# lblQubic/distributed_processor

Hardware: AMD Instinct MI355X
Metric: emulated core-shots/s (config 2: 8-core Ramsey, 100 delays, 1e6 shots/GPU) (higher is better)
Workload: dtype u32; 1 GPU; config2_ramsey_8core_100pt; shots_per_gpu=1000000, lane_order=shot-major, parallelism=shots sharded, 1 GPU(s)

## Files before the change

### distributed_processor_amd/csrc/branch_kernel.h

```cpp

#pragma once

#include <hip/hip_runtime.h>
#include <stdint.h>

#include <type_traits>

#include "lane.h"

namespace dpemu {

namespace {

enum : uint32_t { B_RUN = 0, B_SYNC = 1, B_LUT = 2, B_FIN = 3 };


constexpr uint64_t LATENCY = 0x0003303304646440ull;

template <int OP>
__device__ __forceinline__ uint32_t group_reduce(uint32_t v, uint32_t C)
{
    auto comb = [](uint32_t a, uint32_t b) { return OP == 0 ? (a < b ? a : b) : (a > b ? a : b); };
#define DPP(x, ctrl) ((uint32_t)__builtin_amdgcn_update_dpp(0, (int)(x), (ctrl), 0xF, 0xF, false))
    if (C >= 2) v = comb(v, DPP(v, 0xB1));
    if (C >= 4) v = comb(v, DPP(v, 0x4E));
    if (C >= 8) v = comb(v, DPP(v, 0x141));
    if (C >= 16) v = comb(v, DPP(v, 0x140));
#undef DPP
    for (uint32_t m = 16; m < C; m <<= 1) v = comb(v, (uint32_t)__shfl_xor((int)v, (int)m, 64));
    return v;
}

__device__ __forceinline__ uint32_t wave_min(uint32_t v)
{
    v = group_reduce<0>(v, 16u);
    const uint32_t a = __builtin_amdgcn_readlane(v, 0), b = __builtin_amdgcn_readlane(v, 16);
    const uint32_t c = __builtin_amdgcn_readlane(v, 32), d = __builtin_amdgcn_readlane(v, 48);
    return min(min(a, b), min(c, d));
}

}

template <int FEAT, int CT>
__global__ void __launch_bounds__(BLOCK) branch_kernel(const KParams p)
{
    constexpr bool FPROC = (FEAT & FEAT_FPROC) != 0;
    constexpr bool LUT = (FEAT & FEAT_LUT) != 0;
    constexpr bool XMEAS = FPROC || LUT;
    constexpr bool SYNC = (FEAT & FEAT_SYNC) != 0;
    constexpr bool REGS = (FEAT & FEAT_REGS) != 0;
    constexpr bool PLDS = (FEAT & FEAT_PROG_LDS) != 0;
    constexpr bool DEMOD = (FEAT & FEAT_DEMOD) != 0;
    constexpr int MT = XMEAS ? MEAS_LOOKUP : 1;
    constexpr bool DIRECT = LUT || DEMOD;
    constexpr int NF = LUT ? LUT_FIRE_CAP : 1;

    __shared__ uint32_t s_regs[REGS ? 16 : 1][REGS ? BLOCK : 1];
    __shared__ uint32_t s_mt[MT][BLOCK];
    __shared__ uint32_t s_fire[NF][LUT ? BLOCK : 1];
    __shared__ uint32_t s_pref[PLDS ? BLOCK + 1 : 1];
    __shared__ uint32_t s_scan[BLOCK / 64];
    __shared__ uint32_t s_rof[DEMOD ? 6 : 1][DEMOD ? BLOCK : 1];
    extern __shared__ uint4 s_dyn[];
    uint4 *const s_prog = s_dyn;
    uint32_t *const s_hist = reinterpret_cast<uint32_t *>(s_dyn + (PLDS ? p.prog_lds_words : 0u));

    clear_hist_next(p);
    const uint32_t tid = threadIdx.x;
    const uint32_t C = CT ? (uint32_t)CT : p.C;
    const uint32_t log2C = CT ? (uint32_t)__builtin_ctz(CT) : p.log2C;
    const uint32_t pos = blockIdx.x * BLOCK + tid;
    const bool valid = pos < p.n_lanes;
    const uint32_t core = pos & (C - 1);
    const uint32_t spos = pos >> log2C;
    const uint32_t lane = out_lane(p, spos, core);
    const uint64_t shot = p.shot_begin + spos;
    const uint32_t wl = tid & 63;
    const uint32_t leader_tid = tid & ~(C - 1);
    const uint32_t n_lanes = p.n_lanes, max_cycles = p.max_cycles;

    uint32_t nprog = 0, grp = 0, prog = 0, base = 0;
    if (valid) {
        grp = shot_group(p, spos);
        prog = p.prog_table[(uint64_t)grp * C + core];
        base = p.offsets[prog];
        nprog = p.n_instr[prog];
    }
    if constexpr (PLDS) {
        const uint32_t b = stage_programs(p, s_prog, s_pref, s_scan, spos, core);
        if (valid) base = b;
    }
    const bool cmd_major = !PLDS && p.fetch_stride != 1u;
    const uint32_t fetch_off = cmd_major ? prog : base, k_max = cmd_major ? p.max_len : nprog;
    const uint32_t thr_core = valid ? p.p1_thr[core] : 0u;
    if constexpr (DEMOD) {
        const uint4 h = valid ? p.ro_hdr[prog] : make_uint4(0u, 0u, 0u, 0u);
        s_rof[0][tid] = h.x; s_rof[1][tid] = h.y; s_rof[2][tid] = h.z; s_rof[3][tid] = h.w;
        s_rof[4][tid] = ro_freq(p, h.x, h.y, 0u);
        s_rof[5][tid] = ro_freq(p, h.z, h.w, 0u);
    }
    if (p.hist_lds) {
        for (uint32_t i = tid; i < HIST_LDS_MAX; i += BLOCK) s_hist[i] = 0;
        __syncthreads();
    }
    if constexpr (REGS) {
#pragma unroll
        for (int r = 0; r < 16; r++) s_regs[r][tid] = 0;
    }
    if constexpr (XMEAS) {
#pragma unroll
        for (int m = 0; m < MT; m++) s_mt[m][tid] = INF32;
    }
    uint64_t lut_valid = 0, lut_addr = 0;
    uint32_t lut_last_fire = INF32, nfire = 0, lut_cur = 0;

    uint32_t mode = valid ? B_RUN : B_FIN;
    uint32_t ip = 0, t = 0, qoff = 0xFFFFFFFFu;
    uint32_t pe = 0, pp = 0, pa = 0;
    uint32_t wait_d = 0, status = 0, flags = 0, t_end = 0;
    uint32_t n_ev = 0, n_tr = 0, n_meas = 0, n_exec = 0, meas_bits = 0, last_bit = 0;
    const bool is_part = SYNC ? (((p.sync_mask >> core) & 1ull) != 0) : false;
    uint4 *const ev_lane = p.events + lane;
    uint4 pend0 = make_uint4(0u, 0u, 0u, 0u), pend1 = pend0;
    uint32_t n_st = 0;
    RoDrive ro_d{0u, 0u, 0u};
    uint32_t ro_tref = 0, ro_ltv = 0;

    auto emit = [&](bool ok, uint32_t te, uint32_t kind) __attribute__((always_inline)) {
        if (ok) {
            if (DIRECT && n_ev < p.event_cap && p.events)
                st_rec<ST_WB>(&ev_lane[(uint64_t)n_ev * n_lanes], event_record(te, pe, pp, pa, kind));
            if (!DIRECT && n_ev < p.event_cap && p.events) {
                const uint4 rec = event_record(te, pe, pp, pa, kind);
                const bool full = n_ev - n_st == 2u;
                if (full) st_rec<ST_WB>(&ev_lane[(uint64_t)n_st * n_lanes], pend0);
                pend0 = sel4(full, pend1, pend0);
                n_st += full ? 1u : 0u;
                const bool first = n_ev == n_st;
                pend0 = sel4(first, rec, pend0);
                pend1 = sel4(first, pend1, rec);
            }
            n_ev++;
            if constexpr (DEMOD) {
                if (kind == 1u) ro_tref = te;
                if (kind == 0u && ((pe >> 24) & 3u) == p.ro_drv_elem)
                    ro_d = RoDrive{te, pp & 0x03FFFFFFu, (pa & 0xFFFFu) | (((pe >> 12) & 0xFFFu) << 16) | 0x80000000u};
            }
            if (kind == 0u && ((pe >> 24) & 3u) == p.meas_elem) {
                uint32_t bit, tv;
                if constexpr (DEMOD) {
                    int2 a;
                    const uint32_t fi_lo = (pp >> 17) & 0x1FFu, fi_d = (ro_d.pp >> 17) & 0x1FFu;
                    const uint32_t f_lo = fi_lo ? ro_freq(p, s_rof[2][tid], s_rof[3][tid], fi_lo) : s_rof[5][tid];
                    const uint32_t f_d = fi_d ? ro_freq(p, s_rof[0][tid], s_rof[1][tid], fi_d) : s_rof[4][tid];
                    bit = demod_readout(p, shot, core, n_meas, thr_core, te, pe, pp, ro_d, ro_tref, f_lo, f_d, a);
                    tv = demod_valid(p, te, pe, ro_ltv);
                    ro_ltv = tv;
                    if (p.acc && n_meas < p.meas_cap) p.acc[(uint64_t)n_meas * n_lanes + lane] = a;
                } else {
                    bit = meas_bit(p, shot, core, n_meas, thr_core, pa, pe);
                    tv = te + p.meas_latency;
                }
                if constexpr (XMEAS) {
                    if (n_meas < (uint32_t)MT) s_mt[n_meas < (uint32_t)MT ? n_meas : 0u][tid] = (tv << 1) | bit;
                }
                if (p.meas && n_meas < p.meas_cap) p.meas[(uint64_t)n_meas * n_lanes + lane] = make_uint2(tv, bit);
                meas_bits |= (n_meas < 32u ? bit : 0u) << (n_meas & 31u);
                last_bit = bit;
                n_meas++;
            }
        }
    };

    auto emit_trace = [&](bool ok, uint32_t tt, uint32_t addr, uint32_t val) __attribute__((always_inline)) {
        if (ok) {
            if (n_tr < p.trace_cap && p.trace) p.trace[(uint64_t)n_tr * n_lanes + lane] = make_uint4(tt, addr, val, 0u);
            n_tr++;
        }
    };

    auto meas_lookup = [&](uint32_t q_tid, uint32_t d) -> uint32_t {
        static_assert(MEAS_LOOKUP % 2 == 0, "slots read in pairs");
        uint32_t res = 0;
#pragma unroll 1
        for (int m = 0; m + 1 < MT; m += 2) {
            const uint32_t e0 = s_mt[m][q_tid], e1 = s_mt[m + 1][q_tid];
            if ((e0 >> 1) > d) break;
            res = e0 & 1u;
            if ((e1 >> 1) > d) break;
            res = e1 & 1u;
        }
        return res;
    };

    auto sync_maxkey = [&]() -> uint32_t {
        uint32_t key = mode == B_SYNC ? wait_d : t;
        if constexpr (LUT) key = mode == B_LUT ? wait_d + 5u : key;
        key = mode == B_FIN ? INF32 : key;
        return group_reduce<1>(is_part ? key : 0u, C);
    };

    auto reg = [&](uint32_t r) __attribute__((always_inline)) -> uint32_t {
        if constexpr (REGS) return s_regs[r & 15u][tid];
        return 0u;
    };

    auto finish = [&](bool stop, uint32_t st, uint32_t at) __attribute__((always_inline)) {
        status = stop ? st : status;
        t_end = stop ? at : t_end;
        mode = stop ? B_FIN : mode;
    };

    auto flush_rows = [&](bool all) __attribute__((always_inline)) {
        if (DIRECT || !p.events) return;
        const uint32_t ne = min(n_ev, p.event_cap);
        if (!__any(ne > n_st)) return;
        const uint32_t done = all ? INF32 : wave_min(mode == B_FIN ? INF32 : ne);
        const bool f1 = n_st < ne && n_st < done;
        if (!__any(f1)) return;
        const bool f2 = f1 && n_st + 1u < ne && n_st + 1u < done;
        if (f1) st_rec<ST_WB>(&ev_lane[(uint64_t)n_st * n_lanes], pend0);
        if (__any(f2)) {
            if (f2) st_rec<ST_WB>(&ev_lane[(uint64_t)(n_st + 1u) * n_lanes], pend1);
        }
        pend0 = sel4(f1 && !f2, pend1, pend0);
        n_st += (f1 ? 1u : 0u) + (f2 ? 1u : 0u);
    };

    auto iteration = [&](auto first_tag) -> bool {
        constexpr bool FIRST = decltype(first_tag)::value;
        finish(mode == B_RUN && t > max_cycles, ST_MAX_CYCLES, t);
        const bool run = mode == B_RUN;
        const uint4 u = PLDS ? s_prog[fetch_off + min(ip, k_max)]
                             : p.fetch[(uint64_t)min(ip, k_max) * p.fetch_stride + fetch_off];
        const uint32_t op = u.y >> 28;

        bool stall = false;
        if constexpr (FPROC) {
            const bool fp = run && (op == 4u || op == 5u);
            if (__any(fp)) {
                uint32_t bound = run ? t + 2u : INF32;
                if constexpr (SYNC) {
                    if (__any(mode == B_SYNC)) {
                        const uint32_t maxkey = sync_maxkey();
                        if (mode == B_SYNC && is_part && maxkey != INF32) bound = maxkey + p.sync_latency + 5u;
                    }
                }
                const uint32_t gmin = group_reduce<0>(bound, C);
                stall = fp && !((uint64_t)gmin + p.meas_latency > (uint64_t)t);
            }
        }
        const bool go = run && !stall;
        bool sync_rel = false;
        n_exec += go ? 1u : 0u;
        const uint32_t D = t;
        const uint32_t qD = FIRST ? 0u : D + qoff;

        constexpr uint32_t FAST = 0xFF05u | (SYNC ? 0x80u : 0u);
        const bool pcls = (FAST >> op) & 1u;
        {
            const bool pg = go && pcls;
            const bool waits = (0x1200u >> op) & 1u;
            uint32_t wait = u.x - qD;
            bool big = false, dbl = false;
            if constexpr (FIRST) {
                dbl = u.x == 0u;
                const uint64_t w = dbl ? 0ull : 1ull + u.x;
                wait = (uint32_t)w;
                big = (w >> 32) != 0ull;
            }
            const bool late = waits && (big || wait >= 0x80000000u);
            const bool over = waits && (big || wait > max_cycles - D);
            const uint32_t tT = D + (waits ? wait : 0u);
            const bool jmp = op == 2u;
            const bool to_sync = SYNC && pg && op == 7u;
            const bool cont = pg && (((0x1B04u >> op) & 1u) != 0u) && !over;
            if (__any(cont && ((0x300u >> op) & 1u))) {
                uint32_t pe2 = pe, pp2 = pp, pa2 = pa;
                pulse_write(u, pe2, pp2, pa2);
                if (cont && (u.w & UOP_ANY_RS)) {
                    const uint32_t r0 = reg(u.w >> 20);
                    if (u.w & UOP_RS_ENV) pe2 |= r0 & 0xFFFFFFu;
                    if (u.w & UOP_RS_PH) pp2 |= r0 & 0x1FFFFu;
                    if (u.w & UOP_RS_FR) pp2 |= (r0 & 0x1FFu) << 17;
                    if (u.w & UOP_RS_AMP) pa2 = r0 & 0xFFFFu;
                }
                pe = cont ? pe2 : pe;
                pp = cont ? pp2 : pp;
                pa = cont ? pa2 : pa;
            }
            const bool rst = op == 0xBu;
            emit(cont && (op == 9u || rst), rst ? D : tT + 2u, rst ? 1u : 0u);
            if constexpr (FIRST) {
                const bool two = cont && dbl && op == 9u;
                emit(two, tT + 3u, 0u);
                flags |= two ? F_DOUBLE_STROBE : 0u;
            }
            flags |= (pg && late) ? F_LATE : 0u;
            if (__any(pg && !cont && !to_sync)) {
                finish(pg && !cont && !to_sync, over ? ST_MAX_CYCLES : op >= 0xDu ? ST_HUNG_OPCODE : ST_DONE, D);
            }
            wait_d = to_sync ? D : wait_d;
            mode = to_sync ? B_SYNC : mode;
            ip = cont ? (jmp ? (u.z & 0xFFFFu) : ((ip + 1u) & 0xFFFFu)) : ip;
            t = cont ? (jmp ? D + 4u : tT + 3u) : t;
        }
        if (__any(go && !pcls)) {
            const bool sg = go && !pcls;
            const bool is_fp = op == 4u || op == 5u;
            const uint32_t reg0 = reg(u.w >> 20);
            const uint32_t reg1 = reg(u.y >> 4);
            uint32_t data = 0;
            uint32_t R = D + 2u;
            bool lut_wait = false, no_meas = false;
            if constexpr (FPROC) {
                if (__any(sg && is_fp)) {
                    if (sg && is_fp) data = meas_lookup(leader_tid + (((u.z >> 16) & 0xFFu) & (C - 1u)), D);
                }
            }
            if constexpr (LUT) {
                if (__any(sg && is_fp)) {
                    const bool id0 = ((u.z >> 16) & 0xFFu) == 0u;
                    lut_wait = sg && is_fp && !id0;
                    if (sg && is_fp && id0) {
                        uint32_t e = INF32;
#pragma unroll
                        for (int m = MT - 1; m >= 0; m--) {
                            const uint32_t x = s_mt[m][tid];
                            e = (x != INF32 && (x >> 1) >= D + 1u) ? x : e;
                        }
                        no_meas = e == INF32;
                        R = e >> 1;
                        data = e & 1u;
                    }
                }
            }
            const uint32_t in0 = (u.y & 8u) ? reg0 : u.x;
            const uint32_t out = alu_eval(u.y & 7u, in0, op == 6u ? qD : is_fp ? data : reg1);
            const bool absent = (!XMEAS && is_fp) || (!SYNC && op == 7u);
            const bool r_over = XMEAS && is_fp && !lut_wait && !no_meas && R > max_cycles;
            const bool fin = r_over || absent || no_meas;
            const bool cont = sg && !fin;
            const bool to_sync = SYNC && cont && op == 7u;
            const bool to_lut = LUT && cont && lut_wait;
            const bool adv = cont && !to_sync && !to_lut;
            const uint32_t t_next = (is_fp ? R : D) + (uint32_t)((LATENCY >> (4u * op)) & 15u);
            const bool take = op == 2u || ((op == 3u || op == 5u) && (out & 1u));
            const uint32_t ip_next = take ? (u.z & 0xFFFFu) : ((ip + 1u) & 0xFFFFu);
            const bool wr = adv && (op == 1u || op == 4u);
            if constexpr (REGS) {
                if (wr) s_regs[(u.y >> 8) & 15u][tid] = out;
            }
            const bool inc = adv && op == 6u;
            emit_trace(wr || inc, (op == 4u ? R : D) + 3u, inc ? TRACE_QCLK_LOAD : (u.y >> 8) & 15u,
                       inc ? out + 3u : out);
            qoff = inc ? out - D : qoff;
            finish(sg && fin, r_over ? ST_MAX_CYCLES : ST_DEADLOCK, D);
            wait_d = (to_sync || to_lut) ? D : wait_d;
            mode = to_sync ? B_SYNC : to_lut ? B_LUT : mode;
            ip = adv ? ip_next : ip;
            t = adv ? t_next : t;
        }

        if constexpr (SYNC) {
            if (__any(mode == B_SYNC)) {
                const uint32_t maxkey = sync_maxkey();
                const uint64_t b = __ballot(is_part && mode == B_SYNC);
                const uint64_t pm = __ballot(is_part);
                const bool all_arrived = group_bits(b, wl, C) == group_bits(pm, wl, C) && group_bits(pm, wl, C) != 0ull;
                const bool rel = mode == B_SYNC && is_part && all_arrived;
                const uint32_t S = maxkey + p.sync_latency;
                const bool ok = rel && S <= max_cycles;
                emit_trace(ok, S + 2u, TRACE_QCLK_RST, 0u);
                qoff = ok ? 0u - (S + 2u) : qoff;
                ip = ok ? ((ip + 1u) & 0xFFFFu) : ip;
                t = ok ? S + 3u : t;
                mode = ok ? B_RUN : mode;
                finish(rel && !ok, ST_MAX_CYCLES, wait_d);
                sync_rel = rel;
                if constexpr (!LUT)
                    finish(group_bits(__ballot(go || rel), wl, C) == 0ull && mode == B_SYNC, ST_DEADLOCK, wait_d);
            }
        }

        bool lut_rel = false;
        if constexpr (LUT) {
            __builtin_amdgcn_fence(__ATOMIC_SEQ_CST, "wavefront");
            __builtin_amdgcn_wave_barrier();
            if (__any(mode == B_LUT)) {
                uint32_t bound = mode == B_RUN ? t + 2u : mode == B_LUT ? wait_d + 7u : INF32;
                if constexpr (SYNC) {
                    if (__any(mode == B_SYNC)) {
                        const uint32_t maxkey = sync_maxkey();
                        if (mode == B_SYNC && is_part && maxkey != INF32) bound = maxkey + p.sync_latency + 5u;
                    }
                }
                const uint32_t gmin = group_reduce<0>(bound, C);
                const bool any_run_grp = group_bits(__ballot(mode == B_RUN), wl, C) != 0ull;
                uint32_t H = INF32;
                if (any_run_grp && gmin != INF32) {
                    const uint64_t h = (uint64_t)gmin + p.meas_latency - 1u;
                    H = h > INF32 ? INF32 : (uint32_t)h;
                }
                const bool stop_at_fire = !any_run_grp;
                bool fired = false, busy = valid;
                while (__any(busy)) {
                    const uint32_t e = lut_cur < (uint32_t)MT ? s_mt[lut_cur < (uint32_t)MT ? lut_cur : 0u][tid] : INF32;
                    const uint32_t my = e == INF32 ? INF32 : e >> 1;
                    const uint32_t tmin = group_reduce<0>(my, C);
                    busy = busy && tmin != INF32 && tmin <= H;
                    const bool hit = busy && my == tmin;
                    const uint64_t v = group_bits(__ballot(hit), wl, C);
                    const uint64_t mv = group_bits(__ballot(hit && (e & 1u)), wl, C);
                    lut_cur += hit ? 1u : 0u;
                    const bool upd = busy && !(lut_last_fire != INF32 && tmin == lut_last_fire + 1u);
                    const uint64_t nv = lut_valid | v, na = lut_addr | (v & mv);
                    const bool fire = upd && (((uint64_t)p.lut_mask & nv) == (uint64_t)p.lut_mask);
                    if (fire) {
                        if (nfire < (uint32_t)NF) {
                            const uint64_t o = p.lut_table[na & 0xFFu];
                            s_fire[nfire < (uint32_t)NF ? nfire : 0u][tid] = (tmin << 1) | (uint32_t)((o >> core) & 1ull);
                        }
                        lut_last_fire = tmin;
                        nfire++;
                        fired = true;
                    }
                    lut_valid = fire ? 0ull : upd ? nv : lut_valid;
                    lut_addr = fire ? 0ull : upd ? na : lut_addr;
                    busy = busy && !(fire && stop_at_fire);
                }
                const uint32_t nf_grp = nfire;
                const bool grp_fired = fired;
                __builtin_amdgcn_fence(__ATOMIC_SEQ_CST, "wavefront");
                __builtin_amdgcn_wave_barrier();
                if (mode == B_LUT) {
                    const uint32_t n = nf_grp < (uint32_t)NF ? nf_grp : (uint32_t)NF;
                    for (uint32_t k = 0; k < n; k++) {
                        const uint32_t f = s_fire[k][tid], tf = f >> 1;
                        if (tf >= wait_d + 1u) {
                            const uint4 u2 = PLDS ? s_prog[fetch_off + min(ip, k_max)]
                                                  : p.fetch[(uint64_t)min(ip, k_max) * p.fetch_stride + fetch_off];
                            const uint32_t op2 = u2.y >> 28;
                            const uint32_t in0b = (u2.y & 8u) ? reg(u2.w >> 20) : u2.x;
                            const uint32_t outb = alu_eval(u2.y & 7u, in0b, f & 1u);
                            if (tf > max_cycles) {
                                finish(true, ST_MAX_CYCLES, wait_d);
                            } else if (op2 == 4u) {
                                const uint32_t rd = (u2.y >> 8) & 15u;
                                if constexpr (REGS) s_regs[rd][tid] = outb;
                                emit_trace(true, tf + 3u, rd, outb);
                                ip = (ip + 1u) & 0xFFFFu;
                                t = tf + 4u;
                                mode = B_RUN;
                            } else {
                                ip = (outb & 1u) ? (u2.z & 0xFFFFu) : ((ip + 1u) & 0xFFFFu);
                                t = tf + 6u;
                                mode = B_RUN;
                            }
                            lut_rel = true;
                            break;
                        }
                    }
                }
                lut_rel = lut_rel || (grp_fired && tid == leader_tid);
            }
            if (__any(mode == B_SYNC || mode == B_LUT)) {
                const uint64_t pm = __ballot(go || sync_rel || lut_rel);
                finish(group_bits(pm, wl, C) == 0ull && (mode == B_SYNC || mode == B_LUT), ST_DEADLOCK, wait_d);
            }
        }
        if constexpr (XMEAS) {
            __builtin_amdgcn_fence(__ATOMIC_SEQ_CST, "wavefront");
            __builtin_amdgcn_wave_barrier();
        }
        flush_rows(false);
        return __any(mode != B_FIN);
    };

    if (__any(mode != B_FIN) && iteration(std::true_type{})) {
        for (uint32_t iter = 2; iteration(std::false_type{});) {
            if (++iter > p.iter_guard) {
                flags |= mode != B_FIN ? F_GUARD : 0u;
                finish(mode != B_FIN, ST_DEADLOCK, t);
                break;
            }
        }
    }
    flush_rows(true);
    flags |= (n_ev > p.event_cap ? F_EVENT_OVF : 0u) | (n_meas > min(p.meas_cap, MEAS_LOOKUP) ? F_MEAS_OVF : 0u) |
             ((p.trace_cap && n_tr > p.trace_cap) ? F_TRACE_OVF : 0u);

    if (valid && p.summary) {
        const uint32_t qclk_end = t_end == 0u ? 0u : t_end + qoff;
        write_summary(p, lane, t_end, ip, status, flags, n_ev, n_exec, qclk_end, n_meas, meas_bits, n_tr);
    }
    if (valid && p.regs_out) {
#pragma unroll
        for (int r = 0; r < 16; r++) p.regs_out[(uint64_t)r * n_lanes + lane] = reg(r);
    }
    count_outcome(p, s_hist, valid, core, grp, last_bit);
}

template <int F>
static hipError_t launch_branch_f(const KParams &p, uint32_t blocks, hipStream_t stream)
{
    const size_t shmem = ((F & FEAT_PROG_LDS) ? (size_t)p.prog_lds_words * sizeof(uint4) : 0) +
                         (p.hist_lds ? HIST_LDS_MAX * sizeof(uint32_t) : 0);
    if (p.C == 8) hipLaunchKernelGGL((branch_kernel<F, 8>), dim3(blocks), dim3(BLOCK), shmem, stream, p);
    else hipLaunchKernelGGL((branch_kernel<F, 0>), dim3(blocks), dim3(BLOCK), shmem, stream, p);
    return hipGetLastError();
}

}
```

Measured before the change: 55.43 billion core-shots/s.

## Execute up to three fast-class instructions per interpreter iteration

Moves the fast-opcode handling into a reusable lambda and, after the main step, runs up to two extra fast-path instructions for lanes that just continued, so each loop iteration advances more instructions and spends less on per-iteration overhead (finish checks, sync/LUT handling, wave votes). It also narrows the LUT valid/address bitmasks to 32 bits when the core count fits. The cost is larger code and register use plus extra divergence-vote checks, and lanes that finish their extra slots early sit idle while others keep going.

Result: no change. 55.43 billion core-shots/s (median of 4 runs) (+0.0%).

```diff
diff --git a/distributed_processor_amd/csrc/branch_kernel.h b/distributed_processor_amd/csrc/branch_kernel.h
--- a/distributed_processor_amd/csrc/branch_kernel.h
+++ b/distributed_processor_amd/csrc/branch_kernel.h
@@ -54,6 +54,8 @@
     constexpr int MT = XMEAS ? MEAS_LOOKUP : 1;
     constexpr bool DIRECT = LUT || DEMOD;
     constexpr int NF = LUT ? LUT_FIRE_CAP : 1;
+    constexpr uint32_t FAST = 0xFF05u | (SYNC ? 0x80u : 0u);
+    constexpr int SLOTS = 3;
 
     __shared__ uint32_t s_regs[REGS ? 16 : 1][REGS ? BLOCK : 1];
     __shared__ uint32_t s_mt[MT][BLOCK];
@@ -111,7 +113,8 @@
 #pragma unroll
         for (int m = 0; m < MT; m++) s_mt[m][tid] = INF32;
     }
-    uint64_t lut_valid = 0, lut_addr = 0;
+    using lut_bits_t = std::conditional_t<(CT > 0 && CT <= 32), uint32_t, uint64_t>;
+    lut_bits_t lut_valid = 0, lut_addr = 0;
     uint32_t lut_last_fire = INF32, nfire = 0, lut_cur = 0;
 
     uint32_t mode = valid ? B_RUN : B_FIN;
@@ -227,6 +230,56 @@
         n_st += (f1 ? 1u : 0u) + (f2 ? 1u : 0u);
     };
 
+    auto fast_path = [&](auto first_tag, const uint4 u, const uint32_t op, bool pg, uint32_t D,
+                         uint32_t qD) __attribute__((always_inline)) -> bool {
+        constexpr bool FIRST = decltype(first_tag)::value;
+        const bool waits = (0x1200u >> op) & 1u;
+        uint32_t wait = u.x - qD;
+        bool big = false, dbl = false;
+        if constexpr (FIRST) {
+            dbl = u.x == 0u;
+            const uint64_t w = dbl ? 0ull : 1ull + u.x;
+            wait = (uint32_t)w;
+            big = (w >> 32) != 0ull;
+        }
+        const bool late = waits && (big || wait >= 0x80000000u);
+        const bool over = waits && (big || wait > max_cycles - D);
+        const uint32_t tT = D + (waits ? wait : 0u);
+        const bool jmp = op == 2u;
+        const bool to_sync = SYNC && pg && op == 7u;
+        const bool cont = pg && (((0x1B04u >> op) & 1u) != 0u) && !over;
+        if (__any(cont && ((0x300u >> op) & 1u))) {
+            uint32_t pe2 = pe, pp2 = pp, pa2 = pa;
+            pulse_write(u, pe2, pp2, pa2);
+            if (cont && (u.w & UOP_ANY_RS)) {
+                const uint32_t r0 = reg(u.w >> 20);
+                if (u.w & UOP_RS_ENV) pe2 |= r0 & 0xFFFFFFu;
+                if (u.w & UOP_RS_PH) pp2 |= r0 & 0x1FFFFu;
+                if (u.w & UOP_RS_FR) pp2 |= (r0 & 0x1FFu) << 17;
+                if (u.w & UOP_RS_AMP) pa2 = r0 & 0xFFFFu;
+            }
+            pe = cont ? pe2 : pe;
+            pp = cont ? pp2 : pp;
+            pa = cont ? pa2 : pa;
+        }
+        const bool rst = op == 0xBu;
+        emit(cont && (op == 9u || rst), rst ? D : tT + 2u, rst ? 1u : 0u);
+        if constexpr (FIRST) {
+            const bool two = cont && dbl && op == 9u;
+            emit(two, tT + 3u, 0u);
+            flags |= two ? F_DOUBLE_STROBE : 0u;
+        }
+        flags |= (pg && late) ? F_LATE : 0u;
+        if (__any(pg && !cont && !to_sync)) {
+            finish(pg && !cont && !to_sync, over ? ST_MAX_CYCLES : op >= 0xDu ? ST_HUNG_OPCODE : ST_DONE, D);
+        }
+        wait_d = to_sync ? D : wait_d;
+        mode = to_sync ? B_SYNC : mode;
+        ip = cont ? (jmp ? (u.z & 0xFFFFu) : ((ip + 1u) & 0xFFFFu)) : ip;
+        t = cont ? (jmp ? D + 4u : tT + 3u) : t;
+        return cont;
+    };
+
     auto iteration = [&](auto first_tag) -> bool {
         constexpr bool FIRST = decltype(first_tag)::value;
         finish(mode == B_RUN && t > max_cycles, ST_MAX_CYCLES, t);
@@ -256,55 +309,9 @@
         const uint32_t D = t;
         const uint32_t qD = FIRST ? 0u : D + qoff;
 
-        constexpr uint32_t FAST = 0xFF05u | (SYNC ? 0x80u : 0u);
         const bool pcls = (FAST >> op) & 1u;
-        {
-            const bool pg = go && pcls;
-            const bool waits = (0x1200u >> op) & 1u;
-            uint32_t wait = u.x - qD;
-            bool big = false, dbl = false;
-            if constexpr (FIRST) {
-                dbl = u.x == 0u;
-                const uint64_t w = dbl ? 0ull : 1ull + u.x;
-                wait = (uint32_t)w;
-                big = (w >> 32) != 0ull;
-            }
-            const bool late = waits && (big || wait >= 0x80000000u);
-            const bool over = waits && (big || wait > max_cycles - D);
-            const uint32_t tT = D + (waits ? wait : 0u);
-            const bool jmp = op == 2u;
-            const bool to_sync = SYNC && pg && op == 7u;
-            const bool cont = pg && (((0x1B04u >> op) & 1u) != 0u) && !over;
-            if (__any(cont && ((0x300u >> op) & 1u))) {
-                uint32_t pe2 = pe, pp2 = pp, pa2 = pa;
-                pulse_write(u, pe2, pp2, pa2);
-                if (cont && (u.w & UOP_ANY_RS)) {
-                    const uint32_t r0 = reg(u.w >> 20);
-                    if (u.w & UOP_RS_ENV) pe2 |= r0 & 0xFFFFFFu;
-                    if (u.w & UOP_RS_PH) pp2 |= r0 & 0x1FFFFu;
-                    if (u.w & UOP_RS_FR) pp2 |= (r0 & 0x1FFu) << 17;
-                    if (u.w & UOP_RS_AMP) pa2 = r0 & 0xFFFFu;
-                }
-                pe = cont ? pe2 : pe;
-                pp = cont ? pp2 : pp;
-                pa = cont ? pa2 : pa;
-            }
-            const bool rst = op == 0xBu;
-            emit(cont && (op == 9u || rst), rst ? D : tT + 2u, rst ? 1u : 0u);
-            if constexpr (FIRST) {
-                const bool two = cont && dbl && op == 9u;
-                emit(two, tT + 3u, 0u);
-                flags |= two ? F_DOUBLE_STROBE : 0u;
-            }
-            flags |= (pg && late) ? F_LATE : 0u;
-            if (__any(pg && !cont && !to_sync)) {
-                finish(pg && !cont && !to_sync, over ? ST_MAX_CYCLES : op >= 0xDu ? ST_HUNG_OPCODE : ST_DONE, D);
-            }
-            wait_d = to_sync ? D : wait_d;
-            mode = to_sync ? B_SYNC : mode;
-            ip = cont ? (jmp ? (u.z & 0xFFFFu) : ((ip + 1u) & 0xFFFFu)) : ip;
-            t = cont ? (jmp ? D + 4u : tT + 3u) : t;
-        }
+        bool cont0 = false;
+        if (FIRST || __any(go && pcls)) cont0 = fast_path(first_tag, u, op, go && pcls, D, qD);
         if (__any(go && !pcls)) {
             const bool sg = go && !pcls;
             const bool is_fp = op == 4u || op == 5u;
@@ -360,6 +367,25 @@
             mode = to_sync ? B_SYNC : to_lut ? B_LUT : mode;
             ip = adv ? ip_next : ip;
             t = adv ? t_next : t;
+        }
+
+        if constexpr (SLOTS >= 2) {
+            bool more = cont0;
+#pragma unroll
+            for (int s = 1; s < SLOTS; s++) {
+                if (!__any(more)) break;
+                flush_rows(false);
+                finish(more && t > max_cycles, ST_MAX_CYCLES, t);
+                const uint4 u2 = PLDS ? s_prog[fetch_off + min(ip, k_max)]
+                                      : p.fetch[(uint64_t)min(ip, k_max) * p.fetch_stride + fetch_off];
+                const uint32_t op2 = u2.y >> 28;
+                const bool pg2 = more && mode == B_RUN && ((FAST >> op2) & 1u);
+                more = false;
+                if (__any(pg2)) {
+                    n_exec += pg2 ? 1u : 0u;
+                    more = fast_path(std::false_type{}, u2, op2, pg2, t, t + qoff);
+                }
+            }
         }
 
         if constexpr (SYNC) {
@@ -425,8 +451,8 @@
                         nfire++;
                         fired = true;
                     }
-                    lut_valid = fire ? 0ull : upd ? nv : lut_valid;
-                    lut_addr = fire ? 0ull : upd ? na : lut_addr;
+                    lut_valid = fire ? (lut_bits_t)0 : upd ? (lut_bits_t)nv : lut_valid;
+                    lut_addr = fire ? (lut_bits_t)0 : upd ? (lut_bits_t)na : lut_addr;
                     busy = busy && !(fire && stop_at_fire);
                 }
                 const uint32_t nf_grp = nfire;
```
